# ConsenSys/wittgenstein

Hardware: NVIDIA H100
Metric: simulated-ms/sec, GSFSignature 65,536 nodes (higher is better)
Workload: dtype u64 bitmaps / int32

## Files before the change

### wittgenstein_b200/csrc/wtg_cuda.cu

```cuda
#include <cuda_runtime.h>
#include <unistd.h>

#include <cstdio>
#include <cstdlib>
#include <stdexcept>
#include <string>
#include <vector>

#include "wtg_engine.hpp"

namespace wtg {

#define CUDA_OK(x)                                                                                       \
  do {                                                                                                   \
    cudaError_t e_ = (x);                                                                                \
    if (e_ != cudaSuccess) throw std::runtime_error(std::string("CUDA: ") + cudaGetErrorString(e_) + " at " #x); \
  } while (0)

constexpr int SCAN_THREADS = 256;
constexpr int SCAN_ITEMS = 4;
constexpr int SCAN_TILE = SCAN_THREADS * SCAN_ITEMS;

__global__ void k_begin(Dev d, int mode) {
  if (threadIdx.x >= 32) return;
  if (d.ffwd && mode == 1) {
    CoopWarp c;
    tickBeginFfwd(d, c);
  } else if (d.farCap > 0 && !d.ffwd) {
    CoopWarp c;
    tickBeginFar(d, c, mode);
  } else if (threadIdx.x == 0) {
    tickBegin(d, mode);
  }
}
__global__ void k_end(Dev d, int mode) {
  if (threadIdx.x == 0) tickEnd(d, mode);
}

__device__ __forceinline__ void listAppend(const Dev& d, bool active, int n, int* cnt, int* list, u64* words = nullptr, u64 word = 0) {
  CoopWarp c;
  unsigned m = c.ballot(active);
  if (!m) return;
  int stripe = ((blockIdx.x * blockDim.x + threadIdx.x) >> 5) & (ARENA_STRIPES - 1);
  int base = 0;
  if (c.lane() == 0) base = atomicAdd(&cnt[stripe], c.count(m));
  base = c.bcast(base, 0);
  if (active) {
    size_t at = (size_t)stripe * d.listStripeCap + base + c.rank(m);
    list[at] = n;
    if (words) words[at] = word;
  }
// ... 553 lines not shown
template <class PeerT>
__global__ void k_gsf_shuffle(Dev d, int l, u64 s0, const int* liveRank, const u64* rejOrd, int nRej) {
  int n = d.n0 + blockIdx.x * blockDim.x + threadIdx.x;
  if (n < d.n0 + d.nLoc) gsfShuffleLevel<PeerT>(d, n, l, s0, liveRank, rejOrd, nRej);
}

class CudaBackend : public Backend {
 public:
  cudaStream_t st = nullptr;
  cudaStream_t side = nullptr;
  cudaEvent_t forkEv = nullptr, joinEv = nullptr;
  int devId = 0;
  void bind() const { cudaSetDevice(devId); }
  int sms = 132;
  int smemOptin = 0;
  cudaGraphExec_t tickGraph = nullptr;
  const void* graphFor = nullptr;
  bool useGraph = true;
  long long launches = 0;
  long long graphKernels = 0;
  cudaEvent_t tm0 = nullptr, tm1 = nullptr;
  enum ProfSlot { P_BEGIN, P_COND_SCAN, P_DISPATCH_COUNT, P_SCAN_PARTIAL, P_EXCHANGE, P_SCAN_FINAL, P_DISPATCH_SCATTER, P_NODE,
                  P_EMIT, P_MS_COUNT, P_MS_SCAN, P_MS_SCATTER, P_FREE, P_END, P_COND_SCORE, P_COND_SELECT, P_EMIT_PEERS, NK };
  bool profiling = false;
  std::vector<cudaEvent_t> evPool;
  std::vector<int> evKernel;
  size_t evUsed = 0;
  double profMs[NK] = {};
  long long profCnt[NK] = {};
  const char* profNames[NK] = {"k_begin", "k_cond_scan", "k_dispatch_count", "k_scan_partial", "k_exchange", "k_scan_final",
                               "k_dispatch_scatter", "k_node", "k_emit", "k_ms_count", "k_ms_scan", "k_ms_scatter", "k_free",
                               "k_end", "k_cond_score", "k_cond_select", "k_emit_peers"};

  explicit CudaBackend(int requested = -1) {
    int dev = 0;
    const char* e = std::getenv("LOCAL_RANK");
    int cnt = 0;
    CUDA_OK(cudaGetDeviceCount(&cnt));
    if (cnt == 0) throw std::runtime_error("no CUDA device");
    if (e) dev = std::atoi(e) % cnt;
    const char* e2 = std::getenv("WTG_DEVICE");
    if (e2) dev = std::atoi(e2) % cnt;
    if (requested >= 0) {
      if (requested >= cnt) throw std::invalid_argument("CUDA device " + std::to_string(requested) + " does not exist");
      dev = requested;
    }
    CUDA_OK(cudaSetDevice(dev));
// ... 1 lines not shown
    cudaDeviceProp p;
    CUDA_OK(cudaGetDeviceProperties(&p, dev));
    sms = p.multiProcessorCount;
    CUDA_OK(cudaStreamCreateWithFlags(&st, cudaStreamNonBlocking));
    CUDA_OK(cudaStreamCreateWithFlags(&side, cudaStreamNonBlocking));
    CUDA_OK(cudaEventCreateWithFlags(&forkEv, cudaEventDisableTiming));
    CUDA_OK(cudaEventCreateWithFlags(&joinEv, cudaEventDisableTiming));
    CUDA_OK(cudaDeviceGetAttribute(&smemOptin, cudaDevAttrMaxSharedMemoryPerBlockOptin, dev));
    CUDA_OK(cudaFuncSetAttribute(k_ms_count, cudaFuncAttributeMaxDynamicSharedMemorySize, smemOptin));
    CUDA_OK(cudaFuncSetAttribute(k_ms_scatter, cudaFuncAttributeMaxDynamicSharedMemorySize, smemOptin));
    const char* g = std::getenv("WTG_NO_GRAPH");
    if (g && g[0] == '1') useGraph = false;
  }
  ~CudaBackend() override {
    for (void* q : ipcOpened) cudaIpcCloseMemHandle(q);
    if (tickGraph) cudaGraphExecDestroy(tickGraph);
    if (forkEv) cudaEventDestroy(forkEv);
    if (joinEv) cudaEventDestroy(joinEv);
    if (side) cudaStreamDestroy(side);
    if (st) cudaStreamDestroy(st);
  }
  void* alloc(size_t bytes) override {
    bind();
    void* p = nullptr;
    cudaError_t e = cudaMalloc(&p, bytes);
    if (e != cudaSuccess) throw std::runtime_error("cudaMalloc of " + std::to_string(bytes) + " bytes failed: " + cudaGetErrorString(e));
    CUDA_OK(cudaMemsetAsync(p, 0, bytes, st));
    return p;
  }
  void release(void* p) override { cudaFree(p); }
  int deviceId() const override { return devId; }
// ... 55 lines not shown
    bind();
    if (!tm0) {
      CUDA_OK(cudaEventCreate(&tm0));
      CUDA_OK(cudaEventCreate(&tm1));
    }
    CUDA_OK(cudaEventRecord(tm0, st));
  }
  double timerStopMs() override {
    bind();
    CUDA_OK(cudaEventRecord(tm1, st));
    CUDA_OK(cudaEventSynchronize(tm1));
    float ms = 0;
    CUDA_OK(cudaEventElapsedTime(&ms, tm0, tm1));
    return (double)ms;
  }
  void profileEnable(bool on) override {
    sync();
    profiling = on;
    if (on) {
      for (int i = 0; i < NK; ++i) {
        profMs[i] = 0;
        profCnt[i] = 0;
      }
    }
  }
  int profileRead(double* ms, long long* cnt, const char** names, int cap) override {
    sync();
    int k = 0;
    for (int i = 0; i < NK && k < cap; ++i, ++k) {
      ms[k] = profMs[i];
      cnt[k] = profCnt[i];
      names[k] = profNames[i];
    }
    return k;
  }
  void drainProfile() {
    for (size_t i = 0; i < evUsed; ++i) {
      float ms = 0;
      cudaEventElapsedTime(&ms, evPool[2 * i], evPool[2 * i + 1]);
      profMs[evKernel[i]] += ms;
      profCnt[evKernel[i]] += 1;
    }
    evUsed = 0;
  }
  void profBegin(int kid) {
    if (!profiling) return;
    if (evUsed * 2 + 2 > evPool.size()) {
// ... 14 lines not shown
  }
  void profEnd() {
    if (!profiling) return;
    CUDA_OK(cudaEventRecord(evPool[2 * evUsed + 1], st));
    ++evUsed;
  }

  void fork() {
    CUDA_OK(cudaEventRecord(forkEv, st));
    CUDA_OK(cudaStreamWaitEvent(side, forkEv, 0));
  }
  void join() {
    CUDA_OK(cudaEventRecord(joinEv, side));
    CUDA_OK(cudaStreamWaitEvent(st, joinEv, 0));
  }
  void enqueueTick(const Dev& d, int mode) {
    const int wide = sms * 8;
    const size_t msSmem = (size_t)d.msWarps * d.ring * sizeof(int);
    const bool branches = mode == 1 && !profiling && d.G == 1 && (d.proto == PROTO_GSF || d.proto == PROTO_HANDEL);
    cudaStream_t sd = branches ? side : st;
    if (mode != 3) {
      profBegin(P_BEGIN);
      k_begin<<<1, 32, 0, st>>>(d, mode);
      profEnd();
    }
    if (branches) fork();
    if ((d.proto == PROTO_GSF || d.proto == PROTO_HANDEL) && mode != 3) {
      const size_t smem8 = d.proto == PROTO_GSF ? (size_t)8 * (size_t)(d.qcap / 32) * sizeof(uint32_t) : 0;
      profBegin(P_COND_SCAN);
      k_cond_mark<<<(d.nLoc + 255) / 256, 256, 0, st>>>(d);
      k_cond_nodes<0><<<ARENA_STRIPES * 19, 256, 0, st>>>(d);
      profEnd();
      profBegin(P_COND_SCORE);
      k_cond_score<<<ARENA_STRIPES * 19, 256, 0, st>>>(d);
      profEnd();
      profBegin(P_COND_SELECT);
      k_cond_nodes<1><<<ARENA_STRIPES * 19, 256, smem8, st>>>(d);
      profEnd();
      launches += 4;
      if (d.proto == PROTO_HANDEL) {
        Dev dd = d;
        dd.scanPartial = d.drawScanPartial;
        profBegin(P_SCAN_PARTIAL);
        k_scan_partial<<<wide, SCAN_THREADS, 0, st>>>(dd, 2);
        profEnd();
        profBegin(P_SCAN_FINAL);
        k_scan_final<<<wide, SCAN_THREADS, 0, st>>>(dd, 2);
        profEnd();
        if (d.G > 1) {
          profBegin(P_EXCHANGE);
          k_hpick_publish<<<sms, 256, 0, st>>>(d);
          k_x_sync<<<1, 32, 0, st>>>(d, 3);
          profEnd();
          profBegin(P_COND_SELECT);
          k_hpick_xcheck<<<sms, 256, 0, st>>>(d);
          k_hpick_xapply<<<sms, 256, 0, st>>>(d);
          profEnd();
          launches += 5;
        } else {
          profBegin(P_COND_SELECT);
          k_hpick_check<<<sms, 256, 0, st>>>(d);
          k_hpick_apply<<<sms, 256, 0, st>>>(d);
          profEnd();
          launches += 3;
        }
      }
    }
    if (mode != 2 && mode != 3) {
      profBegin(P_DISPATCH_COUNT);
      k_dispatch_count<<<wide, 256, 0, sd>>>(d);
      profEnd();
      profBegin(P_SCAN_PARTIAL);
      k_scan_partial<<<wide, SCAN_THREADS, 0, sd>>>(d, 0);
      profEnd();
      profBegin(P_SCAN_FINAL);
      k_scan_final<<<wide, SCAN_THREADS, 0, sd>>>(d, 0);
      profEnd();
      profBegin(P_DISPATCH_SCATTER);
      k_dispatch_scatter<<<wide, 256, 0, sd>>>(d);
      profEnd();
      if (branches) join();
      profBegin(P_NODE);
      k_node_msgs<<<(d.nLoc + 255) / 256, 256, 0, st>>>(d);
      k_node_tasks<<<ARENA_STRIPES * 19, 256, 0, st>>>(d);
      if (d.proto == PROTO_CASPER) {
        k_casper_fixups<<<1, 32, 0, st>>>(d);
        launches += 1;
      }
      profEnd();
      launches += 6;
    }
    profBegin(P_SCAN_PARTIAL);
    k_scan_partial<<<wide, SCAN_THREADS, 0, st>>>(d, 1);
    profEnd();
    profBegin(P_SCAN_FINAL);
    k_scan_final<<<wide, SCAN_THREADS, 0, st>>>(d, 1);
    profEnd();
    if (d.G > 1) {
      profBegin(P_EXCHANGE);
      k_x1_publish<<<sms * 2, 256, 0, st>>>(d);
      k_x_sync<<<1, 32, 0, st>>>(d, 0);
      k_x1_totals<<<1, 1, 0, st>>>(d);
      k_x1_offsets<<<sms * 2, 256, 0, st>>>(d);
      profEnd();
      launches += 4;
// ... 18 lines not shown
      k_emit_peers<<<sms * 8, 128, 0, st>>>(d);
      profEnd();
      launches += 1;
    }
    if (d.G > 1) {
      profBegin(P_EXCHANGE);
      k_x_sync<<<1, 32, 0, st>>>(d, 1);
      k_x2_ingest<<<sms * 4, 256, 0, st>>>(d);
      launches += 2;
      if (d.allCap > 0) {
        k_x_all_build<<<d.allWarps / 4, 128, 0, st>>>(d);
        launches += 1;
      }
      profEnd();
    }
    if (branches) fork();
    profBegin(P_MS_COUNT);
    k_ms_count<<<sms * 2, d.msWarps * 32, msSmem, st>>>(d);
    profEnd();
    profBegin(P_MS_SCAN);
    k_ms_scan<<<(d.ring + 127) / 128, 128, 0, st>>>(d);
    profEnd();
    profBegin(P_MS_SCATTER);
    k_ms_scatter<<<sms * 2, d.msWarps * 32, msSmem, st>>>(d);
    profEnd();
    const bool pooled = d.proto == PROTO_GSF || d.proto == PROTO_HANDEL;
    if (pooled) {
      profBegin(P_FREE);
      k_free<<<ARENA_STRIPES * 2, 256, 0, sd>>>(d);
      profEnd();
    }
    if (branches) join();
    profBegin(P_END);
    k_end<<<1, 1, 0, st>>>(d, mode);
    profEnd();
    launches += pooled ? 9 : 8;
  }
  void configure(const Dev& d) {
    const size_t msSmem = (size_t)d.msWarps * d.ring * sizeof(int);
    if (msSmem > (size_t)smemOptin) throw std::runtime_error("time ring too large for the multisplit's shared-memory histogram");
  }
  void tick(const Dev& d, int mode) override {
    bind();
    configure(d);
    enqueueTick(d, mode);
    CUDA_OK(cudaGetLastError());
  }
  void ticks(const Dev& d, int count) override {
    bind();
    configure(d);
    if (!useGraph || profiling || count < 4) {
      for (int i = 0; i < count; ++i) enqueueTick(d, 1);
      CUDA_OK(cudaGetLastError());
      return;
    }
    if (!tickGraph || graphFor != (const void*)d.ctl) {
      if (tickGraph) cudaGraphExecDestroy(tickGraph);
      cudaGraph_t g;
      long long before = launches;
      CUDA_OK(cudaStreamBeginCapture(st, cudaStreamCaptureModeThreadLocal));
      enqueueTick(d, 1);
      CUDA_OK(cudaStreamEndCapture(st, &g));
      graphKernels = launches - before;
      launches = before;
      CUDA_OK(cudaGraphInstantiate(&tickGraph, g, 0));
      cudaGraphDestroy(g);
      graphFor = (const void*)d.ctl;
    }
    for (int i = 0; i < count; ++i) CUDA_OK(cudaGraphLaunch(tickGraph, st));
    launches += graphKernels * count;
  }
  void gsfInitNodes(const Dev& d) override {
    bind();
    k_gsf_init_nodes<<<(d.nLoc + 255) / 256, 256, 0, st>>>(d);
    CUDA_OK(cudaGetLastError());
  }
  void rngCandidates(const Dev& d, unsigned long long s0, unsigned long long count, int maxBound,
                     std::vector<unsigned long long>& out) override {
    bind();
    const u64 chunk = 16384;
    u64 threads = (count + chunk - 1) / chunk;
    int cap = (int)std::min<u64>((u64)1 << 26, count / 1024 + (1 << 16));
    u64* dOut = nullptr;
    int* dCnt = nullptr;
    CUDA_OK(cudaMalloc(&dOut, (size_t)cap * sizeof(u64)));
// ... 40 lines not shown
```

### wittgenstein_b200/csrc/wtg_engine.hpp

```cpp
#pragma once
#include <chrono>
#include <cstdio>
#include <functional>
#include <thread>
#include <cstdlib>
#include <cstring>
#include <memory>
#include <string>
#include <vector>

#include "wtg_host.hpp"
#include "wtg_logic.cuh"
#include "wtg_types.h"

namespace wtg {

struct GsfParams {
  int nodeCount, threshold, pairingTime, timeoutPerLevelMs, periodDurationMs, acceleratedCallsCount, nodesDown;
};

struct SfParams {
  int nodeCount, threshold, pairingTime, signatureSize, replyTimeout, candidateCount;
};

// ... 20 lines not shown
};

struct Backend {
  virtual ~Backend() {}
  virtual void* alloc(size_t bytes) = 0;
  virtual void release(void* p) = 0;
  virtual void upload(void* dst, const void* src, size_t bytes) = 0;
  virtual void download(void* dst, const void* src, size_t bytes) = 0;
  virtual void sync() = 0;
  virtual void tick(const Dev& d, int mode) = 0;
  virtual void ticks(const Dev& d, int count) {
    for (int i = 0; i < count; ++i) tick(d, 1);
  }
  virtual void timerStart() {}
  virtual double timerStopMs() { return 0.0; }
  virtual void profileEnable(bool) {}
  virtual int profileRead(double* ms, long long* launches, const char** names, int cap) { (void)ms; (void)launches; (void)names; (void)cap; return 0; }
  virtual void* allocShared(size_t bytes) { return alloc(bytes); }
  virtual void exportShared(void* p, unsigned char* handle) {
    std::memset(handle, 0, 128);
    std::memcpy(handle + 72, &p, sizeof(p));
  }
  virtual void* importShared(const unsigned char* handle) {
    void* p;
    std::memcpy(&p, handle + 72, sizeof(p));
    return p;
  }
  virtual int deviceId() const { return 0; }
  virtual void gsfInitNodes(const Dev& d) = 0;
  virtual void rngCandidates(const Dev& d, unsigned long long s0, unsigned long long count, int maxBound,
                             std::vector<unsigned long long>& out) = 0;
// ... 229 lines not shown
    d.buckets = dalloc<Ev>((size_t)ring * (size_t)d.bcap);
    d.bucketCount = dalloc<int>(ring);
    d.inboxCnt = dallocNodes<int>();
    d.inboxOff = dallocNodes<int>();
    d.inboxFill = dallocNodes<int>();
    d.nodeTasks = dallocNodes<int>();
    d.listStripeCap = ((NL + 31) / 32 + ARENA_STRIPES - 1) / ARENA_STRIPES * 32 + 32;
    d.dueList = dalloc<int>((size_t)ARENA_STRIPES * d.listStripeCap);
    d.taskList = dalloc<int>((size_t)ARENA_STRIPES * d.listStripeCap);
    d.taskWord = dalloc<unsigned long long>((size_t)ARENA_STRIPES * d.listStripeCap);
    d.inbox = dalloc<unsigned long long>((size_t)d.itemCap);
    d.subCount = dalloc<int>(d.bcap);
    d.itemBase = dalloc<int>(d.bcap);
    d.evSlots = dalloc<int>(d.itemCap);
    d.evDraws = dalloc<int>(d.itemCap);
    d.condFired = dallocNodes<int>();
    d.condDraws = dallocNodes<int>();
    d.condDue = dallocNodes<int>();
    d.workCap = (int)std::max<long long>(1 << 16, 64LL * NL) / ARENA_STRIPES * ARENA_STRIPES;
    d.workList = dalloc<uint32_t>(d.workCap);
    d.condEv = dallocNodes<Ev>();
    d.condTarget = dallocNodes<int>();
    d.slotBase = dalloc<int>((size_t)NL + d.itemCap);
    d.drawBase = dalloc<int>((size_t)NL + d.itemCap);
    d.scanPartial = dalloc<int>(2 * 8192);
    d.desc = dalloc<Desc>(d.descCap);
    d.destScratch = dalloc<uint32_t>(d.destScratchCap);
    d.msWarps = 8;
    while (d.msWarps > 1 && (size_t)d.msWarps * ring * sizeof(int) > 200 * 1024) d.msWarps >>= 1;
    d.msChunks = (d.newEvCap + d.msWarps * MS_SUB_ENVELOPES - 1) / (d.msWarps * MS_SUB_ENVELOPES);
    d.msCount = dalloc<int>((size_t)d.msChunks * (size_t)ring);
    d.freeList = dalloc<uint32_t>(d.freeCap);
    if (sharded()) {
      if (farEnabled && !shardFarOk) throw std::logic_error("this protocol cannot run node-sharded yet (far-future calendar)");
      d.xItemCap = d.itemCap + 1;
      d.stageCapWords = (int)std::min<long long>(0x7fffffffLL, stageWordsWanted);
      d.recCap = d.recCap / shardWorld * shardWorld;
// ... 12 lines not shown
      d.recDest = dalloc<uint32_t>(d.recDestCap);
      d.recArrival = dalloc<int>(d.recDestCap);
    }
    if (farEnabled) {
      d.ffwd = farTicking ? 0 : 1;
      d.farCap = tun.farCap ? (int)tun.farCap : (farTicking ? (int)std::min<long long>(1LL << 26, std::max<long long>(64LL * N + 4096, farWanted))
                                                                  : (int)std::max<long long>(2LL * N + 1024, farWanted));
      d.far = dalloc<FarEv>(d.farCap);
      d.farSel = dalloc<int>(d.farCap);
    }
  }
  int recDestOverride = 0;
  int destScratchOverride = 0;
  bool forceShufSerial = false;
  bool forcePickSerial = false;
  int ringExtra = 0;
  bool farEnabled = false;
  bool farTicking = false;

  Ctl readCtl() {
    Ctl c;
    be->sync();
    be->download(&c, d.ctl, sizeof(Ctl));
    return c;
  }
  void writeCtl(const Ctl& c) { be->upload(d.ctl, &c, sizeof(Ctl)); }

  void checkLatencyBuilder() const {
    if (hm.latKind == LAT_CITY && hm.builder != HostModel::B_AWS)
      throw std::invalid_argument("AwsRegionNetworkLatency needs nodes built by an AWS_* node builder");
// ... 1188 lines not shown
    c.nItems = n;
    c.totalSlots = c.totalDraws = 0;
    c.hReject = 0;
    c.shufReject = 0;
    c.allCnt = (int)allList.size();
    c.nextEvent = 0;
    const int per = d.descCap / ARENA_STRIPES;
    for (int t = 0; t < ARENA_STRIPES; ++t) {
      c.descCnt[t] = std::max(0, std::min(per, n - t * per));
      c.destCnt[t] = c.workCnt[t] = c.dueCnt[t] = c.taskCnt[t] = 0;
    }
    be->upload(d.desc, descs.data(), descs.size() * sizeof(Desc));
    std::vector<int> ones((size_t)n, 1), zerosN((size_t)d.N, 0);
    be->upload(d.evSlots, ones.data(), ones.size() * sizeof(int));
    be->upload(d.evDraws, ones.data(), ones.size() * sizeof(int));
    be->upload(d.condFired, zerosN.data(), zerosN.size() * sizeof(int));
    if (!scratch.empty()) be->upload(d.destScratch, scratch.data(), scratch.size() * sizeof(uint32_t));
    if (!allList.empty()) be->upload(d.allList, allList.data(), allList.size() * sizeof(int));
    {
      std::vector<long long> ms((size_t)d.N), bs((size_t)d.N);
      be->download(ms.data(), d.msgSent, ms.size() * sizeof(long long));
      be->download(bs.data(), d.bytesSent, bs.size() * sizeof(long long));
      for (int i = 0; i < d.N; ++i) {
        ms[(size_t)i] += sent[(size_t)i];
        bs[(size_t)i] += bytes[(size_t)i];
      }
      be->upload(d.msgSent, ms.data(), ms.size() * sizeof(long long));
      be->upload(d.bytesSent, bs.data(), bs.size() * sizeof(long long));
    }
    writeCtl(c);
    be->tick(d, 3);
// ... 267 lines not shown
```

### wittgenstein_b200/csrc/wtg_logic.cuh

```cuda
#pragma once
#include "wtg_types.h"

template <class T, class U>
static inline T wtg_host_fetch_add(T* p, U v) {
  T o = *p;
  *p = (T)(o + (T)v);
  return o;
}
template <class T>
static inline T wtg_host_fetch_max(T* p, T v) {
  T o = *p;
  if (v > o) *p = v;
  return o;
}
template <class T>
static inline T wtg_host_fetch_min(T* p, T v) {
  T o = *p;
  if (v < o) *p = v;
  return o;
}
template <class T>
static inline T wtg_host_cas(T* p, T a, T b) {
  T o = *p;
  if (o == a) *p = b;
// ... 389 lines not shown
  int size = 1 << (l - 1);
  int cV = d.cntVer[n * d.L + l];
  if (cV >= size) return 0;
  Blk b = levelBlock((int)from, l);
  const u64* rowV = d.verified + (size_t)n * d.W64 + b.w0;
  const u64* rowI = d.indivVer + (size_t)n * d.W64 + b.w0;
  const u64* sig = d.pool[l] + (size_t)(uint32_t)pl * (size_t)b.nw;
  int cWI = 0, cWIV = 0, inter = 0, interI = 0;
  poolCounts(c, sig, rowV, rowI, b.nw, cWI, cWIV, inter, interI);
  cWI = c.sum(cWI);
  cWIV = c.sum(cWIV);
  bool bi = c.any(inter != 0), bii = c.any(interI != 0);
  return gsfScoreFrom(l, size, cV, (int)(pl >> 32), bi, cWI, cWIV, bii);
}

WTG_HD bool gsfCondMark(const Dev& d, int n) {
  const Ctl& ctl = *d.ctl;
  bool dueNow = false;
  if (ctl.condMode != 0 && !d.ndown[n]) {
    int ms = d.minStart[n];
    bool due = ctl.condMode == 1 ? (ms <= ctl.tick) : (ms <= ctl.until);
    if (due && d.stamp[n] != ctl.callId) {
      d.stamp[n] = ctl.callId;
      if (d.qLen[n] > 0) {
        dueNow = true;
        d.minStart[n] = ctl.tick + d.pairing[n];
        statAdd(d, n, ST_CONDRUNS, 1ULL);
      }
    }
  }
  d.condDue[n] = dueNow ? 1 : 0;
  if (!dueNow) d.condFired[n] = 0;
  return dueNow;
}

constexpr int COND_UNROLL = 4;
template <class C>
WTG_HD void gsfCondScanQueue(const Dev& d, C& c, int n) {
  int len = d.qLen[n];
  QEntry* q = d.queue + (size_t)n * d.qcap;
  int* qsc = d.qScore + (size_t)n * d.qcap;
  uint32_t* qst = d.qStamp + (size_t)n * d.qcap;
  const uint32_t* ver = d.lvVer + (size_t)n * d.L;
  const int st = n & (ARENA_STRIPES - 1);
  const int per = d.workCap / ARENA_STRIPES;
  int reeval = 0;
  const int myL = c.lane() < d.L ? c.lane() : 0;
// ... 167 lines not shown
    best.meta = (uint32_t)c.bcast((int)best.meta, srcLane);
    best.pl = c.bcast64(best.pl, srcLane);
  }
  if (c.lane() == 0) {
    d.qLen[n] = w;
    if (found) {
      WTG_ATOMIC_ADD(&d.sigChecked[n], 1);
      d.sigQueueSize[n] = w;
      Ev ev;
      ev.kind = EV_TASK;
      ev.to = (uint32_t)n;
      ev.from = best.from;
      ev.meta = best.meta;
      ev.pl = best.pl;
      ev.aux = 0;
      ev.pad = (uint32_t)d.ctl->tick + 1u;
      d.condEv[n] = ev;
      d.condTarget[n] = ctl.tick + pairing;
    }
    d.condFired[n] = found ? 1 : 0;
  }
}

template <class C>
WTG_HD int descAlloc(const Dev& d, C& c, int n, int cnt) {
  int base = 0;
  if (c.lane() == 0) {
    int st = n & (ARENA_STRIPES - 1);
    int per = d.descCap / ARENA_STRIPES;
    int i = WTG_ATOMIC_ADD(&d.ctl->descCnt[st], cnt);
    if (i + cnt > per) {
      setError(d, ERR_DESC_OVERFLOW, i + cnt);
      base = -1;
    } else {
      base = st * per + i;
// ... 1204 lines not shown
      target = -1;
    }
  } else if (target >= 0 && target - ctl.tick >= d.ring) {
    setError(d, ERR_FAR_FUTURE, target);
    target = -1;
  }
  if (shard) {
    if (target >= 0) xStoreEnvelope(d, ownerOf(d, (int)ev.to), g, ev, target);
    return;
  }
  d.newEv[g] = ev;
  d.newTarget[g] = target;
}

WTG_HD void emitCond(const Dev& d, int n) {
  if (!d.condFired[n]) return;
  int g = d.slotBase[n - d.n0];
  if (d.G > 1) g += d.ctl->condXoffS;
  if (g >= d.newEvCap) {
    setError(d, ERR_DESC_OVERFLOW, g);
    return;
  }
  int target = d.condTarget[n];
  if (target - d.ctl->tick >= d.ring) {
    setError(d, ERR_FAR_FUTURE, target);
    target = -1;
  }
  if (d.G > 1 && target < 0) return;
  d.newEv[g] = d.condEv[n];
  d.newTarget[g] = target;
}

WTG_HD void tickBegin(const Dev& d, int mode) {
  Ctl& c = *d.ctl;
  if (mode == 1) {
    c.time += 1;
    c.tick = c.time;
    c.condMode = 1;
    c.nEv = d.bucketCount[c.tick & (d.ring - 1)];
  } else if (mode == 0) {
    c.tick = c.time;
    c.condMode = 0;
    c.nEv = d.bucketCount[c.tick & (d.ring - 1)];
  } else {
    c.tick = c.time + 1;
    c.condMode = 2;
    c.nEv = 0;
  }
  for (int t = 0; t < ARENA_STRIPES; ++t) {
    c.descCnt[t] = 0;
    c.destCnt[t] = 0;
    c.workCnt[t] = 0;
    c.dueCnt[t] = 0;
    c.taskCnt[t] = 0;
  }
  c.nItems = 0;
  c.totalSlots = 0;
  c.totalDraws = 0;
  c.hReject = 0;
  c.allCnt = 0;
  c.shufReject = 0;
  c.peerCnt = 0;
  if (c.nEv > c.maxBucket) c.maxBucket = c.nEv;
  if (d.G > 1) {
    c.xseq += 1;
    c.nEvGlobal = 0;
    for (int q = 0; q < MAX_SHARDS; ++q) c.stageTop[q] = 0;
  }
}
template <class C>
WTG_HD void tickBeginFar(const Dev& d, C& c, int mode) {
  if (mode != 2) farMigrate(d, c, mode == 1 ? d.ctl->time + 1 : d.ctl->time);
  c.sync();
  if (c.lane() == 0) tickBegin(d, mode);
  c.sync();
}
WTG_HD void tickEnd(const Dev& d, int mode) {
  Ctl& c = *d.ctl;
  c.rng = lcgAdvance(d.jumpA, d.jumpC, c.rng, (u64)c.totalDraws);
  c.statDraws += (unsigned long long)c.totalDraws;
  c.statEvents += (unsigned long long)c.nItems;
  if ((d.G > 1 ? c.nEvGlobal : c.nEv) > 0) {
    c.callId += 1;
    c.didSomething = 1;
  }
  if (mode != 2 && mode != 3) d.bucketCount[c.tick & (d.ring - 1)] = 0;
  for (int t = 0; t < ARENA_STRIPES; ++t) c.freeCnt[t] = 0;
  if (d.proto == PROTO_CASPER && d.G > 1 && d.cg->createdThisTick > 1) setError(d, ERR_UNSUPPORTED, 4);
  if (d.G > 1 && d.allCap > 0 && mode != 3) c.allSeq = (int)(((unsigned)c.allSeq + (unsigned)xAllTotal(d)) & 0x3fffffffu);
  if (d.proto == PROTO_GSF && (c.tick & 15) == 0)
    for (int l = INLINE_MAX_LEVEL + 1; l < d.L; ++l) {
      int f = 0;
      for (int t = 0; t < POOL_STRIPES; ++t) f += c.poolFreeCnt[l][t];
      if (f < c.poolMinFree[l]) c.poolMinFree[l] = f;
    }
}
WTG_HD void freeApply(const Dev& d, int i) {
  uint32_t w = d.freeList[i];
  freeDirect(d, (int)(w >> 27), w & 0x7FFFFFFu);
}
WTG_HD int stripedIndex(const int* cnt, int per, int t) {
  for (int s = 0; s < ARENA_STRIPES; ++s) {
    int c = cnt[s];
    if (c > per) c = per;
    if (t < c) return s * per + t;
    t -= c;
  }
  return -1;
}
WTG_HD int stripedTotal(const int* cnt, int per) {
// ... 78 lines not shown
    p.a = d.condDraws[d.n0 + j];
    p.b = 0;
    return p;
  }
  if (which == 0) {
    int nEv = d.ctl->nEv;
    if (j < nEv) {
      p.a = d.subCount[j];
      p.b = 0;
    } else {
      p.a = 0;
      p.b = d.inboxCnt[d.n0 + j - nEv];
    }
  } else {
    if (j < d.nLoc) {
      p.a = d.condFired[d.n0 + j];
      p.b = d.condDraws[d.n0 + j];
    } else {
      p.a = d.evSlots[j - d.nLoc];
      p.b = d.evDraws[j - d.nLoc];
    }
  }
  return p;
}
WTG_HD int scanCount(const Dev& d, int which) { return which == 2 ? d.nLoc : which == 0 ? d.ctl->nEv + d.nLoc : d.nLoc + d.ctl->nItems; }
WTG_HD void scanStore(const Dev& d, int which, int j, Pair ex) {
  if (which == 2) {
    d.hDrawBase[d.n0 + j] = ex.a;
    return;
  }
  if (which == 0) {
// ... 26 lines not shown
```

### wittgenstein_b200/csrc/wtg_types.h

```cpp
#pragma once
#include <stdint.h>

#if defined(__CUDACC__)
#define WTG_HD __host__ __device__ __forceinline__
#else
#define WTG_HD inline
#endif

namespace wtg {

constexpr int POOL_STRIPES = 64;
constexpr int ARENA_STRIPES = 64;
constexpr int MS_SUB_ENVELOPES = 256;
constexpr int MAX_LEVELS = 24;
constexpr int MAX_ACC = 16;
constexpr int INLINE_MAX_LEVEL = 7;
constexpr int MAX_DIST = 1144;
constexpr int MAX_SHARDS = 8;

enum : int { PROTO_NONE = 0, PROTO_PINGPONG = 1, PROTO_GSF = 2, PROTO_SANFERMIN = 3, PROTO_HANDEL = 4, PROTO_CASPER = 5, PROTO_CAPPOS = 6,
             PROTO_SLUSH = 7, PROTO_SNOWFLAKE = 8, PROTO_P2PFLOOD = 9 };

enum : uint32_t {
  EV_MSG = 0,
// ... 182 lines not shown
  int taskCnt[ARENA_STRIPES];
  int xseq;
  int nEvGlobal;
  int condXoffS, condXoffD;
  int allCondS, allCondD;
  int stageTop[MAX_SHARDS];
  int xRecTop[MAX_SHARDS];
  int xRecDestTop[MAX_SHARDS];
  int tieCnt;
  int allSeq;
  int xNext, xAfter;
  int poolMinFree[MAX_LEVELS];
  int poolFreeCnt[MAX_LEVELS][POOL_STRIPES];
  long long serialPasses;
  int peerCnt;
};

enum : int {
  ST_DELIVERIES = 0, ST_TASKS, ST_CONDRUNS, ST_EVALENTRIES, ST_EVALWORDS, ST_UPDATES, ST_CYCLES, ST_SENDS, ST_MULTISENDS,
  ST_SENDWORDS, ST_EVALPOOL, ST_UPDATEWORDS, ST_MAXQUEUE, ST_MAXINBOX, ST_COUNT = 16
};
constexpr int STAT_SLOTS = 1024;

enum : int {
  ERR_NONE = 0,
  ERR_BUCKET_OVERFLOW = 1,
  ERR_QUEUE_OVERFLOW = 2,
  ERR_POOL_EXHAUSTED = 3,
  ERR_FAR_FUTURE = 4,
  ERR_DESC_OVERFLOW = 5,
// ... 57 lines not shown
  int* dueList;
  int* taskList;
  unsigned long long* taskWord;
  int listStripeCap;
  unsigned long long* inbox;
  int* subCount;
  int* itemBase;
  int* evSlots;
  int* evDraws;
  int* condDue;
  uint32_t* workList;
  int* condFired;
  int* condDraws;
  Ev* condEv;
  int* condTarget;
  int* slotBase;
  int* drawBase;
  int* scanPartial;
  Desc* desc;
  uint32_t* destScratch;
  Ev* newEv;
  int* newTarget;
  int* msCount;
  MultiRec* rec;
  uint32_t* recDest;
  int* recArrival;
  uint32_t* freeList;
  int ffwd;
  int farCap;
  FarEv* far;
// ... 88 lines not shown
  int* minStart;
  uint32_t* stamp;
  int* pairing;
  int* qLen;
  int* sigChecked;
  int* sigQueueSize;
  QEntry* queue;
  int* qScore;
  uint32_t* qStamp;
  uint32_t* lvVer;
  void* peers;
  unsigned long long* pool[MAX_LEVELS];
  uint32_t* poolFree[MAX_LEVELS];
  int poolCap[MAX_LEVELS];
  int forcePickSerial;
  int* drawScanPartial;
  int sampleK, sampleM, sampleB;
  double sampleAK;
  uint8_t* avColor;
  int* avNonce;
  int* avRound;
  uint8_t* avPend;
  uint8_t* avFound;
  int floodMsgs, floodWords;
  int floodResend, floodBetween;
  const uint32_t* peerOff;
  const uint32_t* peerIds;
  int* floodCnt;
  unsigned long long* floodBits;
  int* peerList;
// ... 4 lines not shown
```

### wittgenstein_b200/network.py

```python
import ctypes as C
import threading

import numpy as np

from . import _lib
from ._lib import WtgError


def _p(a, t):
    return a.ctypes.data_as(C.POINTER(t))


_tls = threading.local()


def set_thread_device(device):
    _tls.device = device


class Network:
    def __init__(self, _api=None, device=None, shard=None):
        self.api = _api or _lib.api()
        if device is None:
            device = getattr(_tls, "device", None)
# ... 125 lines not shown

    def stats(self):
        out = np.zeros(26, np.int64)
        self.api.check(self.api.stats(self.h, _p(out, C.c_longlong)))
        keys = ["deliveries", "tasks", "cond_runs", "draws", "eval_entries", "eval_words", "updates", "cycles", "sends",
                "multi_sends", "send_words", "events", "max_queue", "max_bucket", "max_inbox", "rec_top", "rec_dest_top",
                "kernel_launches", "min_pool_free", "init_draws", "ring", "bcap", "qcap", "peer_bits", "update_words", "reevaluated"]
        return dict(zip(keys, out.tolist()))

    def timer_start(self):
        self.api.check(self.api.timer_start(self.h))

    def timer_stop_ms(self):
        return float(self.api.timer_stop_ms(self.h))

    def profile_enable(self, on=True):
        self.api.check(self.api.profile_enable(self.h, 1 if on else 0))

    def profile_read(self):
        cap = 64
        ms = (C.c_double * cap)()
        cnt = (C.c_longlong * cap)()
        names = (C.c_char_p * cap)()
        k = self.api.check(self.api.profile_read(self.h, ms, cnt, names, cap))
        return {names[i].decode(): (ms[i], cnt[i]) for i in range(k)}
```

Before: 4948.

## Run next tick's GSF condition evaluation ahead on side stream with double-buffered state

For GSF single-device runs, the condition-evaluation kernels for tick t+1 are launched on a side stream during tick t, after message delivery. They overlap with the tick's scan, multi-send and free kernels. Condition outputs (fired, event, target) are double-buffered by tick parity, and separate condTick/condCall control fields decouple the look-ahead from the current tick. Ticks are captured into several graph shapes (first/middle/last/plain), which adds complexity and a risk of ordering hazards if cond reads state still being modified.

```diff
diff --git a/wittgenstein_b200/csrc/wtg_cuda.cu b/wittgenstein_b200/csrc/wtg_cuda.cu
--- a/wittgenstein_b200/csrc/wtg_cuda.cu
+++ b/wittgenstein_b200/csrc/wtg_cuda.cu
@@ -21,20 +21,23 @@
 constexpr int SCAN_ITEMS = 4;
 constexpr int SCAN_TILE = SCAN_THREADS * SCAN_ITEMS;
 
-__global__ void k_begin(Dev d, int mode) {
+__global__ void k_begin(Dev d, int mode, bool condAhead) {
   if (threadIdx.x >= 32) return;
   if (d.ffwd && mode == 1) {
     CoopWarp c;
     tickBeginFfwd(d, c);
   } else if (d.farCap > 0 && !d.ffwd) {
     CoopWarp c;
-    tickBeginFar(d, c, mode);
+    tickBeginFar(d, c, mode, condAhead);
   } else if (threadIdx.x == 0) {
-    tickBegin(d, mode);
-  }
-}
-__global__ void k_end(Dev d, int mode) {
-  if (threadIdx.x == 0) tickEnd(d, mode);
+    tickBegin(d, mode, condAhead);
+  }
+}
+__global__ void k_end(Dev d, int mode, bool condAhead) {
+  if (threadIdx.x == 0) tickEnd(d, mode, condAhead);
+}
+__global__ void k_cond_begin(Dev d) {
+  if (threadIdx.x == 0) condBegin(d);
 }
 
 __device__ __forceinline__ void listAppend(const Dev& d, bool active, int n, int* cnt, int* list, u64* words = nullptr, u64 word = 0) {
@@ -618,15 +621,18 @@
   void bind() const { cudaSetDevice(devId); }
   int sms = 132;
   int smemOptin = 0;
-  cudaGraphExec_t tickGraph = nullptr;
+  enum { SHAPE_PLAIN, SHAPE_FIRST, SHAPE_LAST, SHAPE_MIDDLE, NSHAPES };
+  cudaGraphExec_t tickGraph[NSHAPES] = {};
+  long long shapeKernels[NSHAPES] = {};
   const void* graphFor = nullptr;
   bool useGraph = true;
   long long launches = 0;
-  long long graphKernels = 0;
   cudaEvent_t tm0 = nullptr, tm1 = nullptr;
   enum ProfSlot { P_BEGIN, P_COND_SCAN, P_DISPATCH_COUNT, P_SCAN_PARTIAL, P_EXCHANGE, P_SCAN_FINAL, P_DISPATCH_SCATTER, P_NODE,
-                  P_EMIT, P_MS_COUNT, P_MS_SCAN, P_MS_SCATTER, P_FREE, P_END, P_COND_SCORE, P_COND_SELECT, P_EMIT_PEERS, NK };
+                  P_EMIT, P_MS_COUNT, P_MS_SCAN, P_MS_SCATTER, P_FREE, P_END, P_COND_SCORE, P_COND_SELECT, P_EMIT_PEERS,
+                  P_SCAN_A_PARTIAL, P_SCAN_A_FINAL, NK };
   bool profiling = false;
+  bool profSplitScans = false;
   std::vector<cudaEvent_t> evPool;
   std::vector<int> evKernel;
   size_t evUsed = 0;
@@ -634,7 +640,7 @@
   long long profCnt[NK] = {};
   const char* profNames[NK] = {"k_begin", "k_cond_scan", "k_dispatch_count", "k_scan_partial", "k_exchange", "k_scan_final",
                                "k_dispatch_scatter", "k_node", "k_emit", "k_ms_count", "k_ms_scan", "k_ms_scatter", "k_free",
-                               "k_end", "k_cond_score", "k_cond_select", "k_emit_peers"};
+                               "k_end", "k_cond_score", "k_cond_select", "k_emit_peers", "k_scan_a_partial", "k_scan_a_final"};
 
   explicit CudaBackend(int requested = -1) {
     int dev = 0;
@@ -666,7 +672,8 @@
   }
   ~CudaBackend() override {
     for (void* q : ipcOpened) cudaIpcCloseMemHandle(q);
-    if (tickGraph) cudaGraphExecDestroy(tickGraph);
+    for (cudaGraphExec_t g : tickGraph)
+      if (g) cudaGraphExecDestroy(g);
     if (forkEv) cudaEventDestroy(forkEv);
     if (joinEv) cudaEventDestroy(joinEv);
     if (side) cudaStreamDestroy(side);
@@ -752,9 +759,10 @@
     CUDA_OK(cudaEventElapsedTime(&ms, tm0, tm1));
     return (double)ms;
   }
-  void profileEnable(bool on) override {
+  void profileEnable(bool on, bool splitScans) override {
     sync();
     profiling = on;
+    profSplitScans = splitScans;
     if (on) {
       for (int i = 0; i < NK; ++i) {
         profMs[i] = 0;
@@ -764,11 +772,17 @@
   }
   int profileRead(double* ms, long long* cnt, const char** names, int cap) override {
     sync();
+    const int shown = profSplitScans ? NK : P_SCAN_A_PARTIAL;
     int k = 0;
-    for (int i = 0; i < NK && k < cap; ++i, ++k) {
+    for (int i = 0; i < shown && k < cap; ++i, ++k) {
       ms[k] = profMs[i];
       cnt[k] = profCnt[i];
       names[k] = profNames[i];
+      const int a = i == P_SCAN_PARTIAL ? P_SCAN_A_PARTIAL : i == P_SCAN_FINAL ? P_SCAN_A_FINAL : -1;
+      if (!profSplitScans && a >= 0) {
+        ms[k] += profMs[a];
+        cnt[k] += profCnt[a];
+      }
     }
     return k;
   }
@@ -813,72 +827,75 @@
     CUDA_OK(cudaEventRecord(joinEv, side));
     CUDA_OK(cudaStreamWaitEvent(st, joinEv, 0));
   }
-  void enqueueTick(const Dev& d, int mode) {
+  void enqueueCond(const Dev& d, cudaStream_t s) {
+    const int wide = sms * 8;
+    const size_t smem8 = d.proto == PROTO_GSF ? (size_t)8 * (size_t)(d.qcap / 32) * sizeof(uint32_t) : 0;
+    profBegin(P_COND_SCAN);
+    k_cond_mark<<<(d.nLoc + 255) / 256, 256, 0, s>>>(d);
+    k_cond_nodes<0><<<ARENA_STRIPES * 19, 256, 0, s>>>(d);
+    profEnd();
+    profBegin(P_COND_SCORE);
+    k_cond_score<<<ARENA_STRIPES * 19, 256, 0, s>>>(d);
+    profEnd();
+    profBegin(P_COND_SELECT);
+    k_cond_nodes<1><<<ARENA_STRIPES * 19, 256, smem8, s>>>(d);
+    profEnd();
+    launches += 4;
+    if (d.proto == PROTO_HANDEL) {
+      Dev dd = d;
+      dd.scanPartial = d.drawScanPartial;
+      profBegin(P_SCAN_PARTIAL);
+      k_scan_partial<<<wide, SCAN_THREADS, 0, s>>>(dd, 2);
+      profEnd();
+      profBegin(P_SCAN_FINAL);
+      k_scan_final<<<wide, SCAN_THREADS, 0, s>>>(dd, 2);
+      profEnd();
+      if (d.G > 1) {
+        profBegin(P_EXCHANGE);
+        k_hpick_publish<<<sms, 256, 0, s>>>(d);
+        k_x_sync<<<1, 32, 0, s>>>(d, 3);
+        profEnd();
+        profBegin(P_COND_SELECT);
+        k_hpick_xcheck<<<sms, 256, 0, s>>>(d);
+        k_hpick_xapply<<<sms, 256, 0, s>>>(d);
+        profEnd();
+        launches += 5;
+      } else {
+        profBegin(P_COND_SELECT);
+        k_hpick_check<<<sms, 256, 0, s>>>(d);
+        k_hpick_apply<<<sms, 256, 0, s>>>(d);
+        profEnd();
+        launches += 3;
+      }
+    }
+  }
+  void enqueueTick(const Dev& d, int mode, bool ownCond = true, bool nextCond = false) {
     const int wide = sms * 8;
     const size_t msSmem = (size_t)d.msWarps * d.ring * sizeof(int);
     const bool branches = mode == 1 && !profiling && d.G == 1 && (d.proto == PROTO_GSF || d.proto == PROTO_HANDEL);
-    cudaStream_t sd = branches ? side : st;
+    const bool condBranch = branches && ownCond;
+    cudaStream_t sd = condBranch ? side : st;
     if (mode != 3) {
       profBegin(P_BEGIN);
-      k_begin<<<1, 32, 0, st>>>(d, mode);
-      profEnd();
-    }
-    if (branches) fork();
-    if ((d.proto == PROTO_GSF || d.proto == PROTO_HANDEL) && mode != 3) {
-      const size_t smem8 = d.proto == PROTO_GSF ? (size_t)8 * (size_t)(d.qcap / 32) * sizeof(uint32_t) : 0;
-      profBegin(P_COND_SCAN);
-      k_cond_mark<<<(d.nLoc + 255) / 256, 256, 0, st>>>(d);
-      k_cond_nodes<0><<<ARENA_STRIPES * 19, 256, 0, st>>>(d);
-      profEnd();
-      profBegin(P_COND_SCORE);
-      k_cond_score<<<ARENA_STRIPES * 19, 256, 0, st>>>(d);
-      profEnd();
-      profBegin(P_COND_SELECT);
-      k_cond_nodes<1><<<ARENA_STRIPES * 19, 256, smem8, st>>>(d);
-      profEnd();
-      launches += 4;
-      if (d.proto == PROTO_HANDEL) {
-        Dev dd = d;
-        dd.scanPartial = d.drawScanPartial;
-        profBegin(P_SCAN_PARTIAL);
-        k_scan_partial<<<wide, SCAN_THREADS, 0, st>>>(dd, 2);
-        profEnd();
-        profBegin(P_SCAN_FINAL);
-        k_scan_final<<<wide, SCAN_THREADS, 0, st>>>(dd, 2);
-        profEnd();
-        if (d.G > 1) {
-          profBegin(P_EXCHANGE);
-          k_hpick_publish<<<sms, 256, 0, st>>>(d);
-          k_x_sync<<<1, 32, 0, st>>>(d, 3);
-          profEnd();
-          profBegin(P_COND_SELECT);
-          k_hpick_xcheck<<<sms, 256, 0, st>>>(d);
-          k_hpick_xapply<<<sms, 256, 0, st>>>(d);
-          profEnd();
-          launches += 5;
-        } else {
-          profBegin(P_COND_SELECT);
-          k_hpick_check<<<sms, 256, 0, st>>>(d);
-          k_hpick_apply<<<sms, 256, 0, st>>>(d);
-          profEnd();
-          launches += 3;
-        }
-      }
-    }
+      k_begin<<<1, 32, 0, st>>>(d, mode, !ownCond);
+      profEnd();
+    }
+    if (condBranch) fork();
+    if ((d.proto == PROTO_GSF || d.proto == PROTO_HANDEL) && mode != 3 && ownCond) enqueueCond(d, st);
     if (mode != 2 && mode != 3) {
       profBegin(P_DISPATCH_COUNT);
       k_dispatch_count<<<wide, 256, 0, sd>>>(d);
       profEnd();
-      profBegin(P_SCAN_PARTIAL);
+      profBegin(P_SCAN_A_PARTIAL);
       k_scan_partial<<<wide, SCAN_THREADS, 0, sd>>>(d, 0);
       profEnd();
-      profBegin(P_SCAN_FINAL);
+      profBegin(P_SCAN_A_FINAL);
       k_scan_final<<<wide, SCAN_THREADS, 0, sd>>>(d, 0);
       profEnd();
       profBegin(P_DISPATCH_SCATTER);
       k_dispatch_scatter<<<wide, 256, 0, sd>>>(d);
       profEnd();
-      if (branches) join();
+      if (condBranch) join();
       profBegin(P_NODE);
       k_node_msgs<<<(d.nLoc + 255) / 256, 256, 0, st>>>(d);
       k_node_tasks<<<ARENA_STRIPES * 19, 256, 0, st>>>(d);
@@ -888,6 +905,14 @@
       }
       profEnd();
       launches += 6;
+    }
+    const bool pooled = d.proto == PROTO_GSF || d.proto == PROTO_HANDEL;
+    if (nextCond) {
+      fork();
+      k_free<<<ARENA_STRIPES * 2, 256, 0, side>>>(d);
+      k_cond_begin<<<1, 1, 0, side>>>(d);
+      enqueueCond(d, side);
+      launches += 2;
     }
     profBegin(P_SCAN_PARTIAL);
     k_scan_partial<<<wide, SCAN_THREADS, 0, st>>>(d, 1);
@@ -936,7 +961,7 @@
       }
       profEnd();
     }
-    if (branches) fork();
+    if (branches && !nextCond) fork();
     profBegin(P_MS_COUNT);
     k_ms_count<<<sms * 2, d.msWarps * 32, msSmem, st>>>(d);
     profEnd();
@@ -946,17 +971,16 @@
     profBegin(P_MS_SCATTER);
     k_ms_scatter<<<sms * 2, d.msWarps * 32, msSmem, st>>>(d);
     profEnd();
-    const bool pooled = d.proto == PROTO_GSF || d.proto == PROTO_HANDEL;
-    if (pooled) {
+    if (pooled && !nextCond) {
       profBegin(P_FREE);
-      k_free<<<ARENA_STRIPES * 2, 256, 0, sd>>>(d);
+      k_free<<<ARENA_STRIPES * 2, 256, 0, branches ? side : st>>>(d);
       profEnd();
     }
     if (branches) join();
     profBegin(P_END);
-    k_end<<<1, 1, 0, st>>>(d, mode);
+    k_end<<<1, 1, 0, st>>>(d, mode, nextCond);
     profEnd();
-    launches += pooled ? 9 : 8;
+    launches += pooled && !nextCond ? 9 : 8;
   }
   void configure(const Dev& d) {
     const size_t msSmem = (size_t)d.msWarps * d.ring * sizeof(int);
@@ -971,26 +995,38 @@
   void ticks(const Dev& d, int count) override {
     bind();
     configure(d);
+    const bool ahead = d.condAhead != 0 && d.proto == PROTO_GSF && d.G == 1 && !profiling && count > 1;
+    auto shapeOf = [&](int i) { return !ahead ? SHAPE_PLAIN : i == 0 ? SHAPE_FIRST : i == count - 1 ? SHAPE_LAST : SHAPE_MIDDLE; };
+    auto enqueueShape = [&](int shape) { enqueueTick(d, 1, shape == SHAPE_PLAIN || shape == SHAPE_FIRST, shape == SHAPE_FIRST || shape == SHAPE_MIDDLE); };
     if (!useGraph || profiling || count < 4) {
-      for (int i = 0; i < count; ++i) enqueueTick(d, 1);
+      for (int i = 0; i < count; ++i) enqueueShape(shapeOf(i));
       CUDA_OK(cudaGetLastError());
       return;
     }
-    if (!tickGraph || graphFor != (const void*)d.ctl) {
-      if (tickGraph) cudaGraphExecDestroy(tickGraph);
-      cudaGraph_t g;
-      long long before = launches;
-      CUDA_OK(cudaStreamBeginCapture(st, cudaStreamCaptureModeThreadLocal));
-      enqueueTick(d, 1);
-      CUDA_OK(cudaStreamEndCapture(st, &g));
-      graphKernels = launches - before;
-      launches = before;
-      CUDA_OK(cudaGraphInstantiate(&tickGraph, g, 0));
-      cudaGraphDestroy(g);
+    if (graphFor != (const void*)d.ctl) {
+      for (cudaGraphExec_t& g : tickGraph)
+        if (g) {
+          cudaGraphExecDestroy(g);
+          g = nullptr;
+        }
       graphFor = (const void*)d.ctl;
     }
-    for (int i = 0; i < count; ++i) CUDA_OK(cudaGraphLaunch(tickGraph, st));
-    launches += graphKernels * count;
+    for (int i = 0; i < count; ++i) {
+      const int shape = shapeOf(i);
+      if (!tickGraph[shape]) {
+        cudaGraph_t g;
+        long long before = launches;
+        CUDA_OK(cudaStreamBeginCapture(st, cudaStreamCaptureModeThreadLocal));
+        enqueueShape(shape);
+        CUDA_OK(cudaStreamEndCapture(st, &g));
+        shapeKernels[shape] = launches - before;
+        launches = before;
+        CUDA_OK(cudaGraphInstantiate(&tickGraph[shape], g, 0));
+        cudaGraphDestroy(g);
+      }
+      CUDA_OK(cudaGraphLaunch(tickGraph[shape], st));
+      launches += shapeKernels[shape];
+    }
   }
   void gsfInitNodes(const Dev& d) override {
     bind();
diff --git a/wittgenstein_b200/csrc/wtg_engine.hpp b/wittgenstein_b200/csrc/wtg_engine.hpp
--- a/wittgenstein_b200/csrc/wtg_engine.hpp
+++ b/wittgenstein_b200/csrc/wtg_engine.hpp
@@ -58,7 +58,7 @@
   }
   virtual void timerStart() {}
   virtual double timerStopMs() { return 0.0; }
-  virtual void profileEnable(bool) {}
+  virtual void profileEnable(bool, bool) {}
   virtual int profileRead(double* ms, long long* launches, const char** names, int cap) { (void)ms; (void)launches; (void)names; (void)cap; return 0; }
   virtual void* allocShared(size_t bytes) { return alloc(bytes); }
   virtual void exportShared(void* p, unsigned char* handle) {
@@ -318,13 +318,15 @@
     d.itemBase = dalloc<int>(d.bcap);
     d.evSlots = dalloc<int>(d.itemCap);
     d.evDraws = dalloc<int>(d.itemCap);
-    d.condFired = dallocNodes<int>();
+    d.condStride = proto == PROTO_GSF ? d.nLoc : 0;
+    d.condAhead = proto == PROTO_GSF && !sharded() ? condAhead : 0;
+    d.condFired = dalloc<int>((size_t)d.nLoc + d.condStride) - d.n0;
     d.condDraws = dallocNodes<int>();
     d.condDue = dallocNodes<int>();
     d.workCap = (int)std::max<long long>(1 << 16, 64LL * NL) / ARENA_STRIPES * ARENA_STRIPES;
     d.workList = dalloc<uint32_t>(d.workCap);
-    d.condEv = dallocNodes<Ev>();
-    d.condTarget = dallocNodes<int>();
+    d.condEv = dalloc<Ev>((size_t)d.nLoc + d.condStride) - d.n0;
+    d.condTarget = dalloc<int>((size_t)d.nLoc + d.condStride) - d.n0;
     d.slotBase = dalloc<int>((size_t)NL + d.itemCap);
     d.drawBase = dalloc<int>((size_t)NL + d.itemCap);
     d.scanPartial = dalloc<int>(2 * 8192);
@@ -367,6 +369,7 @@
   int destScratchOverride = 0;
   bool forceShufSerial = false;
   bool forcePickSerial = false;
+  int condAhead = 1;
   int ringExtra = 0;
   bool farEnabled = false;
   bool farTicking = false;
@@ -1585,7 +1588,7 @@
     std::vector<int> ones((size_t)n, 1), zerosN((size_t)d.N, 0);
     be->upload(d.evSlots, ones.data(), ones.size() * sizeof(int));
     be->upload(d.evDraws, ones.data(), ones.size() * sizeof(int));
-    be->upload(d.condFired, zerosN.data(), zerosN.size() * sizeof(int));
+    be->upload(d.condFired + condHalf(d, time), zerosN.data(), zerosN.size() * sizeof(int));
     if (!scratch.empty()) be->upload(d.destScratch, scratch.data(), scratch.size() * sizeof(uint32_t));
     if (!allList.empty()) be->upload(d.allList, allList.data(), allList.size() * sizeof(int));
     {
diff --git a/wittgenstein_b200/csrc/wtg_logic.cuh b/wittgenstein_b200/csrc/wtg_logic.cuh
--- a/wittgenstein_b200/csrc/wtg_logic.cuh
+++ b/wittgenstein_b200/csrc/wtg_logic.cuh
@@ -427,23 +427,24 @@
   return gsfScoreFrom(l, size, cV, (int)(pl >> 32), bi, cWI, cWIV, bii);
 }
 
+WTG_HD size_t condHalf(const Dev& d, int tick) { return (size_t)(tick & 1) * (size_t)d.condStride; }
 WTG_HD bool gsfCondMark(const Dev& d, int n) {
   const Ctl& ctl = *d.ctl;
   bool dueNow = false;
   if (ctl.condMode != 0 && !d.ndown[n]) {
     int ms = d.minStart[n];
-    bool due = ctl.condMode == 1 ? (ms <= ctl.tick) : (ms <= ctl.until);
-    if (due && d.stamp[n] != ctl.callId) {
-      d.stamp[n] = ctl.callId;
+    bool due = ctl.condMode == 1 ? (ms <= ctl.condTick) : (ms <= ctl.until);
+    if (due && d.stamp[n] != ctl.condCall) {
+      d.stamp[n] = ctl.condCall;
       if (d.qLen[n] > 0) {
         dueNow = true;
-        d.minStart[n] = ctl.tick + d.pairing[n];
+        d.minStart[n] = ctl.condTick + d.pairing[n];
         statAdd(d, n, ST_CONDRUNS, 1ULL);
       }
     }
   }
   d.condDue[n] = dueNow ? 1 : 0;
-  if (!dueNow) d.condFired[n] = 0;
+  if (!dueNow) d.condFired[condHalf(d, ctl.condTick) + n] = 0;
   return dueNow;
 }
 
@@ -641,11 +642,11 @@
       ev.meta = best.meta;
       ev.pl = best.pl;
       ev.aux = 0;
-      ev.pad = (uint32_t)d.ctl->tick + 1u;
-      d.condEv[n] = ev;
-      d.condTarget[n] = ctl.tick + pairing;
-    }
-    d.condFired[n] = found ? 1 : 0;
+      ev.pad = (uint32_t)ctl.condTick + 1u;
+      d.condEv[condHalf(d, ctl.condTick) + n] = ev;
+      d.condTarget[condHalf(d, ctl.condTick) + n] = ctl.condTick + pairing;
+    }
+    d.condFired[condHalf(d, ctl.condTick) + n] = found ? 1 : 0;
   }
 }
 
@@ -1880,24 +1881,25 @@
 }
 
 WTG_HD void emitCond(const Dev& d, int n) {
-  if (!d.condFired[n]) return;
+  const size_t h = condHalf(d, d.ctl->tick);
+  if (!d.condFired[h + n]) return;
   int g = d.slotBase[n - d.n0];
   if (d.G > 1) g += d.ctl->condXoffS;
   if (g >= d.newEvCap) {
     setError(d, ERR_DESC_OVERFLOW, g);
     return;
   }
-  int target = d.condTarget[n];
+  int target = d.condTarget[h + n];
   if (target - d.ctl->tick >= d.ring) {
     setError(d, ERR_FAR_FUTURE, target);
     target = -1;
   }
   if (d.G > 1 && target < 0) return;
-  d.newEv[g] = d.condEv[n];
+  d.newEv[g] = d.condEv[h + n];
   d.newTarget[g] = target;
 }
 
-WTG_HD void tickBegin(const Dev& d, int mode) {
+WTG_HD void tickBegin(const Dev& d, int mode, bool condAhead = false) {
   Ctl& c = *d.ctl;
   if (mode == 1) {
     c.time += 1;
@@ -1916,9 +1918,15 @@
   for (int t = 0; t < ARENA_STRIPES; ++t) {
     c.descCnt[t] = 0;
     c.destCnt[t] = 0;
-    c.workCnt[t] = 0;
-    c.dueCnt[t] = 0;
+    if (!condAhead) {
+      c.workCnt[t] = 0;
+      c.dueCnt[t] = 0;
+    }
     c.taskCnt[t] = 0;
+  }
+  if (!condAhead) {
+    c.condTick = c.tick;
+    c.condCall = c.callId;
   }
   c.nItems = 0;
   c.totalSlots = 0;
@@ -1935,13 +1943,22 @@
   }
 }
 template <class C>
-WTG_HD void tickBeginFar(const Dev& d, C& c, int mode) {
+WTG_HD void tickBeginFar(const Dev& d, C& c, int mode, bool condAhead = false) {
   if (mode != 2) farMigrate(d, c, mode == 1 ? d.ctl->time + 1 : d.ctl->time);
   c.sync();
-  if (c.lane() == 0) tickBegin(d, mode);
+  if (c.lane() == 0) tickBegin(d, mode, condAhead);
   c.sync();
 }
-WTG_HD void tickEnd(const Dev& d, int mode) {
+WTG_HD void samplePoolMinFree(const Dev& d) {
+  Ctl& c = *d.ctl;
+  if (d.proto == PROTO_GSF && (c.tick & 15) == 0)
+    for (int l = INLINE_MAX_LEVEL + 1; l < d.L; ++l) {
+      int f = 0;
+      for (int t = 0; t < POOL_STRIPES; ++t) f += c.poolFreeCnt[l][t];
+      if (f < c.poolMinFree[l]) c.poolMinFree[l] = f;
+    }
+}
+WTG_HD void tickEnd(const Dev& d, int mode, bool condAhead = false) {
   Ctl& c = *d.ctl;
   c.rng = lcgAdvance(d.jumpA, d.jumpC, c.rng, (u64)c.totalDraws);
   c.statDraws += (unsigned long long)c.totalDraws;
@@ -1954,12 +1971,18 @@
   for (int t = 0; t < ARENA_STRIPES; ++t) c.freeCnt[t] = 0;
   if (d.proto == PROTO_CASPER && d.G > 1 && d.cg->createdThisTick > 1) setError(d, ERR_UNSUPPORTED, 4);
   if (d.G > 1 && d.allCap > 0 && mode != 3) c.allSeq = (int)(((unsigned)c.allSeq + (unsigned)xAllTotal(d)) & 0x3fffffffu);
-  if (d.proto == PROTO_GSF && (c.tick & 15) == 0)
-    for (int l = INLINE_MAX_LEVEL + 1; l < d.L; ++l) {
-      int f = 0;
-      for (int t = 0; t < POOL_STRIPES; ++t) f += c.poolFreeCnt[l][t];
-      if (f < c.poolMinFree[l]) c.poolMinFree[l] = f;
-    }
+  if (!condAhead) samplePoolMinFree(d);
+}
+WTG_HD void condBegin(const Dev& d) {
+  Ctl& c = *d.ctl;
+  samplePoolMinFree(d);
+  c.condTick = c.tick + 1;
+  c.condCall = c.callId + (c.nEv > 0 ? 1u : 0u);
+  c.condMode = 1;
+  for (int t = 0; t < ARENA_STRIPES; ++t) {
+    c.workCnt[t] = 0;
+    c.dueCnt[t] = 0;
+  }
 }
 WTG_HD void freeApply(const Dev& d, int i) {
   uint32_t w = d.freeList[i];
@@ -2068,7 +2091,7 @@
     }
   } else {
     if (j < d.nLoc) {
-      p.a = d.condFired[d.n0 + j];
+      p.a = d.condFired[condHalf(d, d.ctl->tick) + d.n0 + j];
       p.b = d.condDraws[d.n0 + j];
     } else {
       p.a = d.evSlots[j - d.nLoc];
diff --git a/wittgenstein_b200/csrc/wtg_types.h b/wittgenstein_b200/csrc/wtg_types.h
--- a/wittgenstein_b200/csrc/wtg_types.h
+++ b/wittgenstein_b200/csrc/wtg_types.h
@@ -220,6 +220,8 @@
   int poolFreeCnt[MAX_LEVELS][POOL_STRIPES];
   long long serialPasses;
   int peerCnt;
+  int condTick;
+  uint32_t condCall;
 };
 
 enum : int {
@@ -307,6 +309,7 @@
   int* condDraws;
   Ev* condEv;
   int* condTarget;
+  int condStride;
   int* slotBase;
   int* drawBase;
   int* scanPartial;
@@ -425,6 +428,7 @@
   uint32_t* poolFree[MAX_LEVELS];
   int poolCap[MAX_LEVELS];
   int forcePickSerial;
+  int condAhead;
   int* drawScanPartial;
   int sampleK, sampleM, sampleB;
   double sampleAK;
diff --git a/wittgenstein_b200/network.py b/wittgenstein_b200/network.py
--- a/wittgenstein_b200/network.py
+++ b/wittgenstein_b200/network.py
@@ -163,8 +163,8 @@
     def timer_stop_ms(self):
         return float(self.api.timer_stop_ms(self.h))
 
-    def profile_enable(self, on=True):
-        self.api.check(self.api.profile_enable(self.h, 1 if on else 0))
+    def profile_enable(self, on=True, split_scans=False):
+        self.api.check(self.api.profile_enable(self.h, (2 if split_scans else 1) if on else 0))
 
     def profile_read(self):
         cap = 64
```

Result: faster. 5146, median of 6 (+4.0%).
